# lenke182/flood-uav-video-segmentation

Hardware: AMD Instinct MI355X
Metric: segmentation FPS @713x713 (PSPNet-ResNet50 keyframe + linear interp, frame_delta=5) (higher is better)
Workload: dtype f32

## Files before the change

flood_uav_video_segmentation_amd/_lib.py:

```python
import ctypes
import os

import torch

_HERE = os.path.dirname(os.path.abspath(__file__))
LIB_PATH = os.path.join(_HERE, "libfloodseg.so")

c_float_p = ctypes.POINTER(ctypes.c_float)
c_void = ctypes.c_void_p
c_int = ctypes.c_int
c_i64 = ctypes.c_int64
c_f32 = ctypes.c_float


class FsConfig(ctypes.Structure):
    _fields_ = [("arch", c_int), ("layers", c_int), ("classes", c_int), ("patch", c_int), ("d_model", c_int),
                ("n_layers", c_int), ("dec_layers", c_int), ("image_size", c_int), ("flags", c_int), ("winograd_tile", c_int)]


ARCH_PSPNET = 0
ARCH_DEEPLABV3 = 1
ARCH_SEGMENTER = 2
OPT_NO_WINOGRAD = 1
OPT_NO_FUSED_HEAD = 2
# ... 87 lines not shown
    ("dual_conv", c_int, [c_void, c_int, c_void, c_int, c_void, c_void, c_void, c_void] + [c_int] * 12 + [c_void]),
    ("pyramid_pool", c_int, [c_void, c_int, c_void] + [c_int] * 4 + [c_void]),
    ("rowdot_batch", c_int, [c_int] + [c_void] * 6 + [c_int] * 5 + [c_void]),
    ("upsample_into", c_int, [c_void, c_int, c_int, c_void] + [c_int] * 6 + [c_void]),
    ("classifier_nchw", c_int, [c_void, c_int, c_void, c_void, c_void] + [c_int] * 4 + [c_void]),
    ("ppm_term_scratch_floats", ctypes.c_size_t, [c_int] * 3),
    ("ppm_term_classify", c_int, [c_void, c_int] + [c_void] * 7 + [c_int] * 5 + [c_void] * 3 + [c_int, c_void, c_void]),
    ("ppm_head_workspace_floats", ctypes.c_size_t, [c_int] * 3),
    ("ppm_head", c_int, [c_void, c_int, c_void, c_int] + [c_void] * 5 + [c_int] * 5 + [c_void] * 3 + [c_int, c_void, c_void]),
    ("block_match", c_int, [c_void, c_void] + [c_int] * 5 + [c_void, c_void, c_void]),
]

_EXT_HOOKS = [
    ("frame_prepare", c_int, [c_void, c_void, c_void] + [c_int] * 5 + [c_void, c_void, c_void, c_int, c_int, c_void]),
    ("frame_compose", c_int, [c_void, c_int, c_int, c_void, c_int, c_void, c_void, c_void] + [c_int] * 5 + [c_void, c_void, c_void] + [c_int] * 3 + [c_void]),
]
EXT_MAGIC = 0x4653455854414231

_EXT2_HOOKS = [
    ("block_match_modes", c_int, [c_void, c_void] + [c_int] * 7 + [c_void, c_void, c_void, c_void, c_void]),
    ("window_weights", c_int, [c_int, ctypes.POINTER(c_void), c_void, c_void, c_void]),
    ("seg_tail_weighted", c_int, [c_void, c_void, ctypes.POINTER(c_void), ctypes.POINTER(c_void)] + [c_int] * 9 + [c_void] * 4 + [c_int] * 4
     + [c_void, c_void, c_void]),
    ("crops_fuse_weighted", c_int, [c_void, c_void, c_void, c_int, ctypes.POINTER(c_int), ctypes.POINTER(c_int)] + [c_int] * 9
     + [c_void, c_void, c_int, c_int, c_void, c_void, c_void]),
    ("feat_tail_weighted", c_int, [c_void, c_void, c_int, c_int, c_int, ctypes.POINTER(c_void), ctypes.POINTER(c_void), c_int, c_int, c_void, c_int,
                                   c_int, c_int, c_int, c_void, c_void, c_void, c_void]),
    ("mask_confidence", c_int, [c_void] + [c_int] * 4 + [c_void, c_void, c_int, c_int, c_void]),
    ("canvas_confidence", c_int, [c_void] + [c_int] * 4 + [c_void, c_void, c_int, c_int, c_void]),
    ("frame_report", c_int, [c_void, c_void] + [c_int] * 5 + [c_void, c_void]),
    ("mask_regions", c_int, [c_void] + [c_int] * 5 + [c_void, c_void]),
    ("region_table", c_int, [c_void, c_void, c_void] + [c_int] * 6 + [c_void] * 5),
    ("region_filter", c_int, [c_void, c_void, c_void] + [c_int] * 6 + [c_void, c_void, c_void]),
]
EXT2_MAGIC = 0x4653455854414232


class FsTestApi(ctypes.Structure):
    _fields_ = [("size", ctypes.c_size_t)] + [(name, ctypes.CFUNCTYPE(res, *args)) for name, res, args in _HOOKS]


class FsExtApi(ctypes.Structure):
    _fields_ = [("magic", ctypes.c_uint64), ("size", ctypes.c_size_t)] + [(name, ctypes.CFUNCTYPE(res, *args)) for name, res, args in _EXT_HOOKS]


class FsHookTables(ctypes.Structure):
    _fields_ = [("test", FsTestApi), ("ext", FsExtApi)]


class FsExt2Api(ctypes.Structure):
    _fields_ = [("magic", ctypes.c_uint64), ("size", ctypes.c_size_t)] + [(name, ctypes.CFUNCTYPE(res, *args)) for name, res, args in _EXT2_HOOKS]


class FsHookTables2(ctypes.Structure):
    _fields_ = [("base", FsHookTables), ("ext2", FsExt2Api)]


class _Library:

    def __init__(self, cdll):
        self._cdll = cdll
        self._hooks = None
        self._ext = None
        self._ext2 = None

    def __getattr__(self, name):
# ... 108 lines not shown
```

flood_uav_video_segmentation_amd/csrc/conv_igemm.hip:

```cpp
#include "kernels.h"
#include "igemm_epilogue.h"

#include <algorithm>
#include <cstdlib>

namespace fs {

#define FS_DMA_PUBLISH() { __builtin_amdgcn_s_waitcnt(0x0070); __syncthreads(); }
constexpr int conv_split_rows(int BN, int waves) { return (BN / 16 + waves - 1) / waves * waves * 16; }
template <int BM, int BN, bool SPLIT, int WAVES = 4>
constexpr int conv_tile_lds_floats() { return 2 * (BM * 32 + (SPLIT ? 3 * conv_split_rows(BN, WAVES) * 16 : BN * 32)); }

template <int TM>
__device__ __forceinline__ void split_unit(int lvl, int pr, const f32x4 (&raw)[TM][2], float (&rq)[4 * TM][2], u32x4 (&ah)[TM][3], bool pin) {
    const int pi = pr / 4, pe = pr % 4;
    float x0 = lvl == 0 ? raw[pi][pe >> 1][2 * (pe & 1)] : rq[pr][0];
    float x1 = lvl == 0 ? raw[pi][pe >> 1][2 * (pe & 1) + 1] : rq[pr][1];
    unsigned pk = split_round(x0, x1);
    if (pin) asm volatile("" : "+v"(pk));
    ah[pi][lvl][pe] = pk;
    if (lvl < 2) {
        split_residue(pk, x0, x1);
        rq[pr][0] = x0;
        rq[pr][1] = x1;
// ... 294 lines not shown
#undef FS_DMA_ADVANCE
#undef FS_DMA_ALL
#undef FS_FRAGS
#undef FS_MMA

    if constexpr (SPLIT && !DUAL && BN == 96 && TM == 1) {
        const int Dm = p.kv_heads * 64;
        if (p.kv_k && n0 >= Dm) {
            const int kind = n0 >= 2 * Dm ? 2 : 1;
            igemm_epilogue_kv<TN>(acc, sc_n, sh_n, p, kind, em_base, en_base - kind * Dm, en_base < p.Cout, lane);
            return;
        }
    }
    if (!DUAL && p.res) {
        if (p.relu == 1) igemm_epilogue<1, true>(acc, rv, sc_n, sh_n, p, M, em_base, en_base);
        else if (p.relu == 2) igemm_epilogue<2, true>(acc, rv, sc_n, sh_n, p, M, em_base, en_base);
        else igemm_epilogue<0, true>(acc, rv, sc_n, sh_n, p, M, em_base, en_base);
    } else {
        if (p.relu == 1) igemm_epilogue<1, false>(acc, rv, sc_n, sh_n, p, M, em_base, en_base);
        else if (p.relu == 2) igemm_epilogue<2, false>(acc, rv, sc_n, sh_n, p, M, em_base, en_base);
        else igemm_epilogue<0, false>(acc, rv, sc_n, sh_n, p, M, em_base, en_base);
    }
#endif
}

template <int BM, int BN, int WGM = 2, int WGN = 2, bool DUAL = false, bool SPLIT = false>
__global__ __launch_bounds__(64 * WGM * WGN) void conv_igemm_dma_f32(ConvParams p, int tiles_m, int tiles_n) {
#if defined(__HIP_DEVICE_COMPILE__)
    constexpr int PM = 8;
    __shared__ __attribute__((aligned(1024))) float lds[conv_tile_lds_floats<BM, BN, SPLIT, WGM * WGN>()];
    const int nblk = gridDim.x, bid = blockIdx.x;
    const int q = nblk >> 3, rr = nblk & 7, xcd = bid & 7;
    const int lid = (xcd < rr ? xcd * (q + 1) : rr * (q + 1) + (xcd - rr) * q) + (bid >> 3);
    const int per_group = tiles_m * tiles_n;
    const int grp = lid / per_group;
    const int lig = lid - grp * per_group;
    const int panel = lig / (PM * tiles_n);
    const int within = lig - panel * (PM * tiles_n);
    const int prow = min(PM, tiles_m - panel * PM);
    const int m0 = (panel * PM + within % prow) * BM, n0 = (within / prow) * BN;
    p.in += (long long)grp * p.g_in;
    p.wgt += (long long)grp * p.g_wgt;
    if (SPLIT) p.wgt3 = (const char*)p.wgt3 + (long long)grp * p.g_wgt * 2;
    p.out += (long long)grp * p.g_out;
    p.kv_b = grp;
    conv_tile<BM, BN, WGM, WGN, DUAL, SPLIT>(p, m0, n0, lds);
#endif
}

namespace {
struct TileCfg { int bm, bn; const char* name; };
const TileCfg kTiles[7] = {{0, 0, "auto"}, {128, 128, "igemm128x128"}, {128, 64, "igemm128x64"},
                           {64, 64, "igemm64x64"}, {64, 128, "igemm64x128"}, {0, 0, nullptr}, {128, 96, "split128x96"}};
bool tile_id_ok(int tile) { return tile >= 0 && tile <= 6 && tile != 5; }

int pick_tile(const ConvParams& p) {
    const int M = p.B * p.Ho * p.Wo;
    const double eff[7] = {0, 1.00, 0.92, 0.80, 0.92, 0, 0.97};
    int best = 1;
    double best_t = 1e300;
    const int last = p.in2 ? 2 : p.wgt3 ? 3 : 4;
    for (int c = 1; c <= 6; ++c) {
        if (c > last && !(c == 6 && p.wgt3 && !p.in2 && p.Cout % 96 == 0)) continue;
        const int bm = kTiles[c].bm, bn = kTiles[c].bn;
        if (p.Cout < bn && bn > 64) continue;
        const long tiles = (long)cdiv(M, bm) * cdiv(p.Cout, bn) * (p.groups > 1 ? p.groups : 1);
        const long per_cu = (tiles + 255) / 256;
        const double t = (double)per_cu * bm * bn / (eff[c] * (per_cu >= 2 ? 1.0 : 0.8));
        if (t < best_t) { best_t = t; best = c; }
// ... 39 lines not shown
        FS_REQUIRE((p.H2 - 1) / p.stride2 + 1 == p.Ho && (p.W2 - 1) / p.stride2 + 1 == p.Wo, "conv_igemm: second operand %dx%d / stride %d does not give %dx%d",
                   p.H2, p.W2, p.stride2, p.Ho, p.Wo);
        FS_REQUIRE((int64_t)p.B * p.H2 * p.W2 * p.ld_in2 * 4 < (int64_t)1 << 31, "conv_igemm: second operand must be smaller than 2 GiB");
    }
    FS_REQUIRE(p.ld_in % 4 == 0 && p.ld_in >= p.Cin, "conv_igemm: bad ld_in=%d (Cin=%d)", p.ld_in, p.Cin);
    FS_REQUIRE(p.ld_out >= p.Cout, "conv_igemm: bad ld_out=%d (Cout=%d)", p.ld_out, p.Cout);
    FS_REQUIRE(((uintptr_t)p.in & 15) == 0 && ((uintptr_t)p.wgt & 15) == 0, "conv_igemm: unaligned operand");
    FS_REQUIRE(p.Ho == (p.H + 2 * p.pad - p.dil * (p.KH - 1) - 1) / p.stride + 1 &&
               p.Wo == (p.W + 2 * p.pad - p.dil * (p.KW - 1) - 1) / p.stride + 1,
               "conv_igemm: output geometry %dx%d inconsistent with input %dx%d", p.Ho, p.Wo, p.H, p.W);
    FS_REQUIRE(((int64_t)p.B * p.H * p.W * p.ld_in + ((int64_t)p.pad * p.W + p.pad) * p.ld_in) * 4 < (int64_t)1 << 31,
               "conv_igemm: input tensor must be smaller than 2 GiB");
    FS_REQUIRE((int64_t)p.Cout * std::max(p.ld_wgt, p.KH * p.KW * p.Cin + (p.in2 ? p.Cin2 : 0)) * 4 < (int64_t)1 << 31, "conv_igemm: filter bank must be smaller than 2 GiB");
    FS_REQUIRE(p.ld_wgt == 0 || (p.ld_wgt >= p.KH * p.KW * p.Cin + (p.in2 ? p.Cin2 : 0) && p.ld_wgt % 4 == 0), "conv_igemm: bad ld_wgt=%d", p.ld_wgt);
    FS_REQUIRE(p.KH * p.KW <= 32, "conv_igemm: at most 32 filter taps");
    FS_REQUIRE((int64_t)p.B * p.Ho * p.Wo * p.ld_out * 4 < (int64_t)1 << 31 && ((uintptr_t)p.out & 3) == 0,
               "conv_igemm: output tensor must be smaller than 2 GiB");
    FS_REQUIRE(p.res == nullptr || (int64_t)p.B * p.Ho * p.Wo * p.ld_res * 4 < (int64_t)1 << 31, "conv_igemm: residual tensor must be smaller than 2 GiB");
    if (!(p.res == nullptr || p.ld_res >= p.Cout)) return fail("conv_igemm: bad ld_res");
    return 0;
}
}

int launch_conv_igemm(const ConvParams& p, hipStream_t s, int tile) {
    FS_TRY(check_conv_params(p));
    FS_REQUIRE(tile_id_ok(tile), "conv_igemm: tile %d is not 0..4 or 6", tile);
    if (tile == 0) tile = pick_tile(p);
    FS_REQUIRE(tile < 6 || (p.wgt3 && !p.in2), "conv_igemm: tile 6 (128 x 96) exists on the split-operand route only");
    const int M = p.B * p.Ho * p.Wo;
    const int bm = kTiles[tile].bm, bn = kTiles[tile].bn;
    const int tm = cdiv(M, bm), tn = cdiv(p.Cout, bn);
    const int groups = p.groups > 1 ? p.groups : 1;
    FS_REQUIRE(groups == 1 || p.res == nullptr, "conv_igemm: grouped GEMM has no residual input");
    const dim3 grid(tm * tn * groups), block(256);
    if (p.kv_k) {
        const int Dm = p.kv_heads * 64;
        FS_REQUIRE(tile == 6 && p.wgt3 && !p.in2 && !p.res && p.KH == 1 && p.KW == 1 && p.stride == 1 && p.pad == 0 && p.relu == 0,
                   "conv_igemm: the K / V plane epilogue belongs to a plain Linear on the 128 x 96 split tile");
        FS_REQUIRE(p.kv_vt && p.kv_heads >= 1 && Dm % 96 == 0 && p.Cout == 3 * Dm && p.kv_N == M && p.kv_Npad % 32 == 0 && p.kv_Npad >= M &&
                       p.kv_Npad <= tm * bm && (int64_t)3 * p.kv_plane_bytes < (int64_t)1 << 31 &&
                       (int64_t)p.kv_plane_bytes == (int64_t)groups * p.kv_heads * p.kv_Npad * 128 && (((uintptr_t)p.kv_k | (uintptr_t)p.kv_vt) & 15) == 0,
                   "conv_igemm: bad K / V plane geometry (heads %d, tokens %d, padded %d)", p.kv_heads, p.kv_N, p.kv_Npad);
    }
    if (p.wgt3) {
        FS_REQUIRE(((uintptr_t)p.wgt3 & 15) == 0 && p.plane_bytes % 16 == 0 && (int64_t)3 * p.plane_bytes < (int64_t)1 << 31 && ldw_ok(p),
                   "conv_igemm: bad split filter bank (plane_bytes=%u)", p.plane_bytes);
        FS_REQUIRE((int64_t)groups * p.g_wgt * 2 <= (int64_t)p.plane_bytes, "conv_igemm: the groups' filters (%d x %lld) exceed a plane of the split bank", groups, p.g_wgt);
    }
    if (p.in2 && p.wgt3) {
        if (tile == 2) hipLaunchKernelGGL((conv_igemm_dma_f32<128, 64, 4, 1, true, true>), grid, block, 0, s, p, tm, tn);
        else if (tile == 1) hipLaunchKernelGGL((conv_igemm_dma_f32<128, 128, 4, 1, true, true>), grid, block, 0, s, p, tm, tn);
        else return fail("conv_igemm: concatenated-K launches use tile 1 or 2");
        FS_HIP(hipGetLastError());
        return 0;
    }
    if (p.in2) {
        if (tile == 2) hipLaunchKernelGGL((conv_igemm_dma_f32<128, 64, 2, 2, true>), grid, block, 0, s, p, tm, tn);
        else if (tile == 1) hipLaunchKernelGGL((conv_igemm_dma_f32<128, 128, 2, 2, true>), grid, block, 0, s, p, tm, tn);
        else return fail("conv_igemm: concatenated-K launches use tile 1 or 2");
        FS_HIP(hipGetLastError());
        return 0;
    }
    if (p.wgt3) {
        switch (tile) {
            case 1: hipLaunchKernelGGL((conv_igemm_dma_f32<128, 128, 4, 1, false, true>), grid, block, 0, s, p, tm, tn); break;
            case 2: hipLaunchKernelGGL((conv_igemm_dma_f32<128, 64, 4, 1, false, true>), grid, block, 0, s, p, tm, tn); break;
            case 3: hipLaunchKernelGGL((conv_igemm_dma_f32<64, 64, 2, 2, false, true>), grid, block, 0, s, p, tm, tn); break;
// ... 22 lines not shown
```

flood_uav_video_segmentation_amd/csrc/kernels.h:

```cpp
#pragma once
#include "common.h"

namespace fs {

struct ConvParams {
    const float* in;    int ld_in;
    const float* wgt;
    int ld_wgt;
    const float* scale;
    const float* shift;
    const float* res;   int ld_res;
    float* out;         int ld_out;
    int B, H, W, Cin;
    int Ho, Wo, Cout;
    int KH, KW, stride, pad, dil;
    const float* in2;   int ld_in2;
    int Cin2, stride2, H2, W2;
    int relu;
    int res_touch;
    int korder;
    int groups;
    long long g_in, g_wgt, g_out;
    const void* wgt3;
    unsigned plane_bytes;
    unsigned short* kv_k;
    unsigned short* kv_vt;
    int kv_N, kv_Npad, kv_heads;
    unsigned kv_plane_bytes;
    int kv_b;
};
int launch_conv_igemm(const ConvParams& p, hipStream_t s, int tile = 0);
const char* conv_igemm_tile_name(const ConvParams& p, int tile = 0);
int launch_split_bf16x3(const float* w, long long n, void* planes, hipStream_t s);

static inline int conv_out_size(int in, int k, int stride, int pad, int dil) { return (in + 2 * pad - dil * (k - 1) - 1) / stride + 1; }
static inline ConvParams conv2d_params(const float* in, int ld_in, const float* wgt, const float* scale, const float* shift, const float* res, int ld_res,
                                       float* out, int ld_out, int B, int H, int W, int Cin, int Cout, int KH, int KW, int stride, int pad, int dil,
                                       int relu, int korder) {
    ConvParams p{};
    p.in = in; p.ld_in = ld_in; p.wgt = wgt; p.scale = scale; p.shift = shift; p.res = res; p.ld_res = ld_res; p.out = out; p.ld_out = ld_out;
    p.B = B; p.H = H; p.W = W; p.Cin = Cin; p.Cout = Cout;
    p.Ho = conv_out_size(H, KH, stride, pad, dil);
    p.Wo = conv_out_size(W, KW, stride, pad, dil);
    p.KH = KH; p.KW = KW; p.stride = stride; p.pad = pad; p.dil = dil; p.relu = relu; p.korder = korder;
    return p;
}
static inline ConvParams gemm_params(const float* in, int ld_in, const float* w, float* out, int ld_out, int rows, int K, int N) {
    return conv2d_params(in, ld_in, w, nullptr, nullptr, nullptr, 0, out, ld_out, 1, rows, 1, K, N, 1, 1, 1, 0, 1, 0, 0);
}
static inline void attach_planes(ConvParams& p, const void* planes, size_t elems) {
    p.wgt3 = planes;
    p.plane_bytes = (unsigned)(elems * 2);
}

struct FrameSrc {
// ... 252 lines not shown
```

flood_uav_video_segmentation_amd/csrc/net.h:

```cpp
#pragma once
#include <map>
#include <memory>
#include <string>
#include <vector>

#include "../../include/floodseg.h"
#include "kernels.h"

namespace fs {

struct RawTensor {
    float* d = nullptr;
    std::vector<int64_t> shape;
    int64_t numel() const {
        int64_t n = 1;
        for (auto s : shape) n *= s;
        return n;
    }
};

struct WinoBank {
    float* U4 = nullptr;
    float* U6 = nullptr;
    float* U3 = nullptr;
// ... 97 lines not shown
    bool res_touch = true;
    std::map<const float*, std::pair<void*, size_t>> split_banks;
    int device = 0;

    float* buf[4] = {nullptr, nullptr, nullptr, nullptr};
    size_t buf_elems = 0;
    float* small = nullptr;
    size_t small_elems = 0;

    bool profiling = false;
    std::vector<fs::ProfRec> prof;

    int feat_channels() const {
        if (cfg.arch == FS_ARCH_SEGMENTER) return cfg.d_model;
        return cfg.arch == FS_ARCH_PSPNET ? 4096 : 2048;
    }
};

namespace fs {
int net_create(const fs_config* cfg, fs_handle* out);
int net_destroy(fs_handle h);
int check_device(fs_net* h, const char* what);
int net_load_weight(fs_handle h, const char* name, const float* data, const int64_t* shape, int ndim, int on_device,
                    hipStream_t s);
int net_finalize(fs_handle h, hipStream_t s);
int net_feature_shape(fs_handle h, int H, int W, int* C, int* fh, int* fw);
size_t net_workspace_bytes(fs_handle h, int B, int H, int W);
int net_reserve(fs_handle h, int B, int H, int W, hipStream_t s);
size_t net_reserved_bytes(fs_handle h);
int net_encoder(fs_handle h, const FrameSrc& src, int B, int H, int W, float* out_nhwc, hipStream_t s);
int net_segment(fs_handle h, const FrameSrc& src, int B, int H, int W, float* out_nchw, hipStream_t s);
int net_decoder(fs_handle h, const float* feat, int B, int fh, int fw, float* out_nchw, hipStream_t s);
int net_profile_dump(fs_handle h, char* buf, size_t n);

int dev_alloc(fs_net* h, float** p, size_t elems);
int ws_grow(fs_net* h, float** p, size_t* have, size_t need, bool zero);
int split_attach(fs_net* h, const float* bank, size_t elems, hipStream_t s);
void split_use(const fs_net* h, ConvParams& p);

int linear_splits(int K, int N, int rows_per_image, int act, bool split_route);
ConvParams linear_params(const float* in, const float* w, const float* bias, const float* res, float* out, int rows, int K, int N, int act,
                         bool res_touch);
ConvParams linear_splitk_params(const float* in, const float* w, float* part, int rows, int K, int N, int split);
ConvParams linear_qkv_params(const float* in, const float* w, const float* bias, float* out, int B, int tokens, int D, float* planes);
ConvParams dual_conv_params(const float* a, int ld_a, const float* b, int ld_b, const float* wgt, const float* shift, float* out, int ld_out, int B,
                            int Ho, int Wo, int Cin, int Cin2, int H2, int W2, int stride2, int Cout, int relu);
ConvParams ppm_z_params(const float* reduced, const float* zw, float* zbuf, int B, int Cr, int Cout9);
int pyramid_pool(fs_net* h, const float* feat, int ld_feat, float* pooled, int B, int H, int W, int C, const int bins[4], hipStream_t s);
int conv_winograd(fs_net* h, const std::string& name, const float* in, int ld_in, const float* U, const void* U3, unsigned plane_bytes, float* V,
                  float* M, const float* scale, const float* shift, float* out, int ld_out, int B, int H, int W, int Cin, int Cout, int dil,
                  int relu, int mt, hipStream_t s);
int vit_reserve(fs_handle h, int B, int H, int W, hipStream_t s);
int fetch(fs_net* h, const std::string& name, const RawTensor** out);
int prof_begin(fs_net* h, const std::string& name, const char* kernel, double flops, double bytes, hipStream_t s);
int prof_end(fs_net* h, hipStream_t s);
int run_igemm(fs_net* h, const std::string& name, const ConvParams& p, double flops, double bytes, hipStream_t s, int tile = 0);
int vit_finalize(fs_handle h, hipStream_t s);
int vit_feature_shape(fs_handle h, int H, int W, int* C, int* fh, int* fw);
int vit_encoder(fs_handle h, const FrameSrc& src, int B, int H, int W, float* out_tokens, hipStream_t s);
int vit_decoder(fs_handle h, const float* tokens, int B, int gh, int gw, float* out_nchw, hipStream_t s);
}
```

flood_uav_video_segmentation_amd/csrc/net.hip:

```cpp
#include "net.h"

#include <cmath>
#include <cstdarg>
#include <cstring>

namespace fs {

std::string& last_error() {
    static thread_local std::string e;
    return e;
}
int fail(const char* fmt, ...) {
    char buf[1024];
    va_list ap;
    va_start(ap, fmt);
    vsnprintf(buf, sizeof(buf), fmt, ap);
    va_end(ap);
    last_error() = buf;
    return 1;
}

int dev_alloc(fs_net* h, float** p, size_t elems) {
    FS_HIP(hipMalloc(reinterpret_cast<void**>(p), std::max<size_t>(elems, 4) * sizeof(float)));
    h->owned.push_back(*p);
// ... 552 lines not shown
    size_t wino = 0;
    if (h->deep_stem) {
        FS_TRY(reserve_conv(h, h->stem[1], B, g.H1, g.W1, s, &wino));
        FS_TRY(reserve_conv(h, h->stem[2], B, g.H1, g.W1, s, &wino));
    }
    int curH = g.H2, curW = g.W2;
    for (const Bottleneck& blk : h->blocks) {
        FS_TRY(reserve_conv(h, blk.c2, B, curH, curW, s, &wino));
        curH = blk.c2.out_size(curH);
        curW = blk.c2.out_size(curW);
    }
    if (psp) {
        FS_TRY(reserve_conv(h, h->use_fused_head ? h->cls_main : h->cls_conv, B, fh, fw, s, &wino));
        FS_TRY(reserve_conv(h, h->cls_conv, B, fh, fw, s, &wino));
    } else {
        for (int i = 1; i < 4; ++i) FS_TRY(reserve_conv(h, h->aspp[i], B, fh, fw, s, &wino));
        FS_TRY(reserve_conv(h, h->head_conv, B, fh, fw, s, &wino));
    }
    return ws_grow(h, &h->wino_ws, &h->wino_ws_elems, wino, false);
}

size_t net_reserved_bytes(fs_handle h) {
    if (!h) return 0;
    return (4 * h->buf_elems + h->small_elems + h->seg_feat_elems + h->wino_ws_elems + h->vit_ws_elems + h->pos_elems + h->bank_elems) * sizeof(float);
}

ConvParams dual_conv_params(const float* a, int ld_a, const float* b, int ld_b, const float* wgt, const float* shift, float* out, int ld_out, int B,
                            int Ho, int Wo, int Cin, int Cin2, int H2, int W2, int stride2, int Cout, int relu) {
    ConvParams p = conv2d_params(a, ld_a, wgt, nullptr, shift, nullptr, 0, out, ld_out, B, Ho, Wo, Cin, Cout, 1, 1, 1, 0, 1, relu, 0);
    p.in2 = b; p.ld_in2 = ld_b; p.Cin2 = Cin2; p.stride2 = stride2; p.H2 = H2; p.W2 = W2;
    return p;
}

ConvParams ppm_z_params(const float* reduced, const float* zw, float* zbuf, int B, int Cr, int Cout9) {
    const int rows = B * 36;
    ConvParams p = gemm_params(reduced, Cr, zw, zbuf, Cout9, rows, Cr, Cout9);
    p.groups = 4;
    p.g_in = (long long)rows * Cr;
    p.g_wgt = (long long)Cout9 * Cr;
    p.g_out = (long long)rows * Cout9;
    return p;
}

int pyramid_pool(fs_net* h, const float* feat, int ld_feat, float* pooled, int B, int H, int W, int C, const int bins[4], hipStream_t s) {
    size_t pool_off[4];
    {
        size_t po = 0;
        for (int i = 0; i < 4; ++i) {
            pool_off[i] = po;
            po += (size_t)B * bins[i] * bins[i] * C;
        }
    }
    const double bytes = 4.0 * B * H * W * C;
    if (H % 6 == 0 && W % 6 == 0 && bins[0] == 1 && bins[1] == 2 && bins[2] == 3 && bins[3] == 6) {
        FS_TRY(prof_begin(h, "ppm.pool6+combine", "adaptive_avgpool", 0, bytes, s));
        FS_TRY(launch_adaptive_avgpool(feat, ld_feat, pooled + pool_off[3], B, H, W, C, 6, s));
        FS_TRY(launch_ppm_pool_combine(pooled + pool_off[3], pooled + pool_off[0], pooled + pool_off[1], pooled + pool_off[2], B, C, s));
        FS_TRY(prof_end(h, s));
        return 0;
    }
    for (int i = 0; i < 4; ++i) {
        FS_TRY(prof_begin(h, "ppm.pool" + std::to_string(bins[i]), "adaptive_avgpool", 0, bytes, s));
        FS_TRY(launch_adaptive_avgpool(feat, ld_feat, pooled + pool_off[i], B, H, W, C, bins[i], s));
        FS_TRY(prof_end(h, s));
    }
    return 0;
}

namespace {
int pyramid_reduce(fs_net* h, const float* feat, int ld_feat, int B, int H, int W, hipStream_t s) {
    float* pooled = h->small;
    float* reduced = h->small + (size_t)B * 50 * 2048;
    FS_TRY(pyramid_pool(h, feat, ld_feat, pooled, B, H, W, 2048, h->bins, s));
// ... 130 lines not shown
    FS_REQUIRE(out_nchw && B >= 1 && H >= 1 && W >= 1, "fs_segment_forward: bad arguments (B=%d H=%d W=%d)", B, H, W);
    FS_TRY(check_frames(src, B, "fs_segment_forward"));
    int C = 0, fh = 0, fw = 0;
    if (h->cfg.arch != FS_ARCH_PSPNET || !h->use_fused_head) {
        FS_TRY(net_feature_shape(h, H, W, &C, &fh, &fw));
        const size_t need = h->cfg.arch == FS_ARCH_SEGMENTER ? (size_t)B * (fh * fw + 1) * C : (size_t)B * fh * fw * C;
        FS_TRY(ws_grow(h, &h->seg_feat, &h->seg_feat_elems, need, false));
        FS_TRY(net_encoder(h, src, B, H, W, h->seg_feat, s));
        return net_decoder(h, h->seg_feat, B, fh, fw, out_nchw, s);
    }
    FS_REQUIRE(H >= 33 && W >= 33, "fs_segment_forward: bad arguments (B=%d H=%d W=%d)", B, H, W);
    const Geometry g = geometry(h, H, W);
    fh = g.H3;
    fw = g.W3;
    FS_TRY(ensure_workspace(h, std::max(encoder_buf_elems(h, B, H, W), ppm_term_scratch_floats(B, fh, h->cls_main.Cout)), small_elems_for(B)));
    float* feat = nullptr;
    FS_TRY(encoder_core(h, src, B, H, W, nullptr, &feat, s));
    hipStream_t ps = s;
    FS_TRY(pyramid_reduce(h, feat, 2048, B, fh, fw, ps));
    float *T = nullptr, *R = nullptr;
    for (int i = 0; i < 4; ++i)
        if (h->buf[i] != feat) {
            R = T;
            T = h->buf[i];
        }
    FS_REQUIRE(ppm_term_scratch_floats(B, fh, h->cls_main.Cout) <= h->buf_elems, "fs_segment_forward: workspace too small for the pyramid term");
    const int K = h->cfg.classes, O = h->cls_main.Cout;
    const size_t px = (size_t)B * fh * fw;
    float* reduced = h->small + (size_t)B * 50 * 2048;
    float* zbuf = reduced + (size_t)4 * B * 36 * 512;
    const float* Z[4];
    {
        const ConvBN& z = h->ppm_z[0];
        ConvParams p = ppm_z_params(reduced, z.w, zbuf, B, 512, z.Cout);
        split_use(h, p);
        FS_TRY(run_igemm(h, "decoder.0.weight[:, ppm]", p, 2.0 * B * 50 * 512.0 * z.Cout, 4.0 * (4.0 * z.Cout * 512 + B * 50.0 * (512 + z.Cout)), ps));
        for (int i = 0; i < 4; ++i) Z[i] = zbuf + (size_t)i * p.g_out;
    }
    ConvBN raw = h->cls_main;
    raw.scale = raw.shift = nullptr;
    raw.relu = 0;
    FS_TRY(run_conv(h, raw, feat, 2048, B, fh, fw, T, O, nullptr, 0, s));
    FS_TRY(prof_begin(h, "decoder.0.pyramid_term+decoder.4", "ppm_term_classify", 2.0 * px * O * (24.0 + K), 4.0 * px * O, s));
    FS_TRY(launch_ppm_term_classify(T, O, Z, h->bins, R, h->cls_main.scale, h->cls_main.shift, B, fh, fw, O, 1, h->cls_w, h->cls_b, out_nchw, K, s));
    return prof_end(h, s);
}

int net_decoder(fs_handle h, const float* feat, int B, int fh, int fw, float* out_nchw, hipStream_t s) {
    FS_REQUIRE(h && h->finalized, "fs_decoder_forward: network not finalized");
    FS_TRY(check_device(h, "fs_decoder_forward"));
    if (h->cfg.arch == FS_ARCH_SEGMENTER) return vit_decoder(h, feat, B, fh, fw, out_nchw, s);
    FS_REQUIRE(feat && out_nchw && B >= 1 && fh >= 1 && fw >= 1, "fs_decoder_forward: bad arguments");
    const int K = h->cfg.classes;
    const size_t px = (size_t)B * fh * fw;
    if (h->cfg.arch == FS_ARCH_PSPNET) {
        FS_TRY(ensure_workspace(h, px * 512, small_elems_for(B)));
        float* T = h->buf[0];
        FS_TRY(run_conv(h, h->cls_conv, feat, 4096, B, fh, fw, T, 512, nullptr, 0, s));
        FS_TRY(prof_begin(h, "decoder.4", "classifier_nchw", 2.0 * px * 512.0 * K, 4.0 * px * 512.0, s));
        FS_TRY(launch_classifier_nchw(T, 512, h->cls_w, h->cls_b, out_nchw, B, fh * fw, 512, K, s));
        return prof_end(h, s);
    }
    FS_TRY(ensure_workspace(h, px * 1280, small_elems_for(B)));
    float *cat = h->buf[0], *P = h->buf[1], *Q = h->buf[2];
    for (int i = 0; i < 4; ++i) FS_TRY(run_conv(h, h->aspp[i], feat, 2048, B, fh, fw, cat + 256 * i, 1280, nullptr, 0, s));
    float* pooled = h->small;
    float* reduced = h->small + (size_t)B * 2048;
    FS_TRY(prof_begin(h, "aspp.pool", "adaptive_avgpool", 0, 4.0 * px * 2048.0, s));
    if (fh % 6 == 0 && fw % 6 == 0) {
        float* cells = h->small + (size_t)B * 4096;
        float* spare = cells + (size_t)B * 36 * 2048;
        FS_TRY(launch_adaptive_avgpool(feat, 2048, cells, B, fh, fw, 2048, 6, s));
        FS_TRY(launch_ppm_pool_combine(cells, pooled, spare, spare + (size_t)B * 4 * 2048, B, 2048, s));
    } else {
        FS_TRY(launch_adaptive_avgpool(feat, 2048, pooled, B, fh, fw, 2048, 1, s));
    }
    FS_TRY(prof_end(h, s));
    FS_TRY(prof_begin(h, h->aspp_pool.name, "rowdot_1x1", 2.0 * B * 2048.0 * 256.0, 4.0 * 2048.0 * 256.0, s));
// ... 32 lines not shown
```

flood_uav_video_segmentation_amd/csrc/net_ops.hip:

```cpp
#include "interp.h"
#include "kernels.h"
#include "split.h"

#include <type_traits>

namespace fs {

template <int CPT >
__global__ __launch_bounds__(256) void stem_conv_kernel(StemParams p) {
    extern __shared__ __attribute__((aligned(16))) float wlds[];
    const int taps = p.KH * p.KW * 3;
    for (int i = threadIdx.x; i < taps * p.Cout; i += 256) wlds[i] = p.wgt[i];
    __syncthreads();

    const int groups = p.Cout / CPT;
    const int ppb = 256 / groups;
    const int cg = threadIdx.x % groups;
    const int M = p.B * p.Ho * p.Wo;
    const int m = blockIdx.x * ppb + threadIdx.x / groups;
    if (m >= M) return;
    const int hw = p.Ho * p.Wo;
    const int b = m / hw;
    const int rem = m - b * hw;
    const int oy = rem / p.Wo, ox = rem - oy * p.Wo;
// ... 376 lines not shown
__global__ __launch_bounds__(256) void ppm_pool_combine_kernel(const float* __restrict__ cell_mean , float* __restrict__ out1,
                                                               float* __restrict__ out2, float* __restrict__ out3, int B, int C) {
    const int64_t total = (int64_t)B * C;
    for (int64_t i = (int64_t)blockIdx.x * 256 + threadIdx.x; i < total; i += (int64_t)gridDim.x * 256) {
        const int c = (int)(i % C), b = (int)(i / C);
        const float* m = cell_mean + (size_t)b * 36 * C + c;
        float s3[9], s2[4] = {0.f, 0.f, 0.f, 0.f}, s1 = 0.f;
#pragma unroll
        for (int k = 0; k < 9; ++k) s3[k] = 0.f;
#pragma unroll
        for (int y = 0; y < 6; ++y)
#pragma unroll
            for (int x = 0; x < 6; ++x) {
                const float v = m[(size_t)(y * 6 + x) * C];
                s3[(y / 2) * 3 + x / 2] += v;
                s2[(y / 3) * 2 + x / 3] += v;
                s1 += v;
            }
#pragma unroll
        for (int k = 0; k < 9; ++k) out3[((size_t)b * 9 + k) * C + c] = s3[k] * 0.25f;
#pragma unroll
        for (int k = 0; k < 4; ++k) out2[((size_t)b * 4 + k) * C + c] = s2[k] * (1.f / 9.f);
        out1[(size_t)b * C + c] = s1 * (1.f / 36.f);
    }
}

int launch_ppm_pool_combine(const float* cell_mean, float* out1, float* out2, float* out3, int B, int C, hipStream_t s) {
    const int64_t total = (int64_t)B * C;
    hipLaunchKernelGGL(ppm_pool_combine_kernel, dim3((unsigned)cdiv64(total, 256)), dim3(256), 0, s, cell_mean, out1, out2, out3, B, C);
    FS_HIP(hipGetLastError());
    return 0;
}

template <int KV >
__global__ __launch_bounds__(256) void rowdot_1x1_kernel(RowdotBatch pb, int ld_in, int ld_out, int K, int N, int relu) {
    const RowdotProblem& q = pb.p[blockIdx.z];
    const int lane = threadIdx.x & 63;
    const int n = blockIdx.x * 4 + (threadIdx.x >> 6);
    if (n >= N) return;
    const int M = q.M;
    const int per = (M + gridDim.y - 1) / gridDim.y;
    const int m_begin = blockIdx.y * per, m_end = min(M, (int)(blockIdx.y + 1) * per);
    if (m_begin >= m_end) return;
    f32x4 w[KV];
#pragma unroll
    for (int i = 0; i < KV; ++i) w[i] = *reinterpret_cast<const f32x4*>(q.wgt + (size_t)n * K + (i * 64 + lane) * 4);
    const float sc = q.scale ? q.scale[n] : 1.f, sh = q.shift ? q.shift[n] : 0.f;
    for (int m = m_begin; m < m_end; ++m) {
        float acc = 0.f;
#pragma unroll
        for (int i = 0; i < KV; ++i) {
            const f32x4 x = *reinterpret_cast<const f32x4*>(q.in + (size_t)m * ld_in + (i * 64 + lane) * 4);
            acc += x[0] * w[i][0] + x[1] * w[i][1] + x[2] * w[i][2] + x[3] * w[i][3];
        }
#pragma unroll
        for (int off = 32; off > 0; off >>= 1) acc += __shfl_xor(acc, off, 64);
        if (lane == 0) {
            float y = acc * sc + sh;
            if (relu) y = fmaxf(y, 0.f);
            q.out[(size_t)m * ld_out + n] = y;
        }
    }
}

int launch_rowdot_1x1_batch(const RowdotBatch& pb, int nprob, int ld_in, int ld_out, int K, int N, int relu, hipStream_t s) {
    FS_REQUIRE(K % 256 == 0 && K <= 4096, "rowdot_1x1: K=%d must be a multiple of 256 and <= 4096", K);
    FS_REQUIRE(nprob >= 1 && nprob <= 4, "rowdot_1x1: 1..4 problems per launch");
    int mmax = 1;
    for (int i = 0; i < nprob; ++i) mmax = std::max(mmax, pb.p[i].M);
    const dim3 grid(cdiv(N, 4), std::max(1, std::min(12, mmax / 6)), nprob), block(256);
#define FS_ROWDOT(KV)                                                                                             \
    case KV:                                                                                                      \
        hipLaunchKernelGGL((rowdot_1x1_kernel<KV>), grid, block, 0, s, pb, ld_in, ld_out, K, N, relu);            \
        break;
    switch (K / 256) {
        FS_ROWDOT(1) FS_ROWDOT(2) FS_ROWDOT(3) FS_ROWDOT(4) FS_ROWDOT(5) FS_ROWDOT(6) FS_ROWDOT(7) FS_ROWDOT(8)
        FS_ROWDOT(9) FS_ROWDOT(10) FS_ROWDOT(11) FS_ROWDOT(12) FS_ROWDOT(13) FS_ROWDOT(14) FS_ROWDOT(15) FS_ROWDOT(16)
        default: return fail("rowdot_1x1: unsupported K");
    }
#undef FS_ROWDOT
    FS_HIP(hipGetLastError());
    return 0;
}

int launch_rowdot_1x1(const float* in, int ld_in, const float* wgt, const float* scale, const float* shift, float* out,
                      int ld_out, int M, int K, int N, int relu, hipStream_t s) {
    RowdotBatch pb{};
    pb.p[0] = RowdotProblem{in, wgt, scale, shift, out, M};
    return launch_rowdot_1x1_batch(pb, 1, ld_in, ld_out, K, N, relu, s);
}

int launch_upsample_into(const float* in, int hi, int wi, float* out, int ld_out, int B, int Ho, int Wo, int C,
                         int align_corners, hipStream_t s) {
    FS_REQUIRE(C % 4 == 0 && ld_out % 4 == 0 && ((uintptr_t)out & 15) == 0, "upsample_into: C/ld_out must be multiples of 4");
    return launch_resize_bilinear_nhwc(in, C, B, C, hi, wi, out, ld_out, Ho, Wo, align_corners, s, 256 * 32);
}

__global__ __launch_bounds__(256) void classifier_nchw_kernel(const float* __restrict__ in, int ld_in, const float* __restrict__ wgt,
                                                              const float* __restrict__ bias, float* __restrict__ out, int B,
                                                              int HW, int C, int K) {
    extern __shared__ __attribute__((aligned(16))) float wl[];
    for (int i = threadIdx.x; i < K * C; i += 256) wl[i] = wgt[i];
    __syncthreads();
    const int l16 = threadIdx.x & 15;
    const int64_t M = (int64_t)B * HW;
    const int64_t m = (int64_t)blockIdx.x * 16 + (threadIdx.x >> 4);
    const int64_t mc = m < M ? m : M - 1;
    const float* x = in + (size_t)mc * ld_in;
    for (int k0 = 0; k0 < K; k0 += 8) {
        float acc[8];
// ... 332 lines not shown
```

Before: 1244.

## Size PPM grouped GEMM per-bin rows and restructure rowdot 1x1 kernel

The pyramid-pooling grouped GEMM now carries per-group row counts (B*bin^2), so each bin launches only the row tiles it needs instead of padding every group to 36 rows. The rowdot 1x1 kernel now computes several output channels and two rows per wave, reusing each input load across channels. It splits rows into fixed chunks across problems and stages results in LDS for vectorised stores. A poison hook is also added for testing that skipped rows are never read. The cost is more register pressure in rowdot and extra index arithmetic in the igemm tile mapping.

```diff
diff --git a/flood_uav_video_segmentation_amd/_lib.py b/flood_uav_video_segmentation_amd/_lib.py
--- a/flood_uav_video_segmentation_amd/_lib.py
+++ b/flood_uav_video_segmentation_amd/_lib.py
@@ -143,6 +143,7 @@
     ("mask_regions", c_int, [c_void] + [c_int] * 5 + [c_void, c_void]),
     ("region_table", c_int, [c_void, c_void, c_void] + [c_int] * 6 + [c_void] * 5),
     ("region_filter", c_int, [c_void, c_void, c_void] + [c_int] * 6 + [c_void, c_void, c_void]),
+    ("pyramid_poison", c_int, [c_void, c_int, c_void]),
 ]
 EXT2_MAGIC = 0x4653455854414232
 
diff --git a/flood_uav_video_segmentation_amd/csrc/conv_igemm.hip b/flood_uav_video_segmentation_amd/csrc/conv_igemm.hip
--- a/flood_uav_video_segmentation_amd/csrc/conv_igemm.hip
+++ b/flood_uav_video_segmentation_amd/csrc/conv_igemm.hip
@@ -350,9 +350,17 @@
     const int nblk = gridDim.x, bid = blockIdx.x;
     const int q = nblk >> 3, rr = nblk & 7, xcd = bid & 7;
     const int lid = (xcd < rr ? xcd * (q + 1) : rr * (q + 1) + (xcd - rr) * q) + (bid >> 3);
-    const int per_group = tiles_m * tiles_n;
-    const int grp = lid / per_group;
-    const int lig = lid - grp * per_group;
+    int grp, lig;
+    if (p.g_rows[0] > 0) {
+        const int t0 = ((p.g_rows[0] + BM - 1) / BM) * tiles_n, t1 = ((p.g_rows[1] + BM - 1) / BM) * tiles_n, t2 = ((p.g_rows[2] + BM - 1) / BM) * tiles_n;
+        grp = lid < t0 ? 0 : lid < t0 + t1 ? 1 : lid < t0 + t1 + t2 ? 2 : 3;
+        lig = lid - (grp > 0 ? t0 : 0) - (grp > 1 ? t1 : 0) - (grp > 2 ? t2 : 0);
+        tiles_m = (((grp == 0 ? p.g_rows[0] : grp == 1 ? p.g_rows[1] : grp == 2 ? p.g_rows[2] : p.g_rows[3]) + BM - 1) / BM);
+    } else {
+        const int per_group = tiles_m * tiles_n;
+        grp = lid / per_group;
+        lig = lid - grp * per_group;
+    }
     const int panel = lig / (PM * tiles_n);
     const int within = lig - panel * (PM * tiles_n);
     const int prow = min(PM, tiles_m - panel * PM);
@@ -458,7 +466,16 @@
     const int tm = cdiv(M, bm), tn = cdiv(p.Cout, bn);
     const int groups = p.groups > 1 ? p.groups : 1;
     FS_REQUIRE(groups == 1 || p.res == nullptr, "conv_igemm: grouped GEMM has no residual input");
-    const dim3 grid(tm * tn * groups), block(256);
+    int row_tiles = tm * groups;
+    if (p.g_rows[0] > 0) {
+        FS_REQUIRE(groups >= 2 && groups <= 4 && !p.kv_k, "conv_igemm: per-group row counts belong to a plain grouped GEMM of 2..4 groups");
+        row_tiles = 0;
+        for (int g = 0; g < 4; ++g) {
+            FS_REQUIRE(g < groups ? p.g_rows[g] >= 1 && p.g_rows[g] <= M : p.g_rows[g] == 0, "conv_igemm: group %d has %d rows of %d", g, p.g_rows[g], M);
+            row_tiles += cdiv(p.g_rows[g], bm);
+        }
+    }
+    const dim3 grid(row_tiles * tn), block(256);
     if (p.kv_k) {
         const int Dm = p.kv_heads * 64;
         FS_REQUIRE(tile == 6 && p.wgt3 && !p.in2 && !p.res && p.KH == 1 && p.KW == 1 && p.stride == 1 && p.pad == 0 && p.relu == 0,
diff --git a/flood_uav_video_segmentation_amd/csrc/kernels.h b/flood_uav_video_segmentation_amd/csrc/kernels.h
--- a/flood_uav_video_segmentation_amd/csrc/kernels.h
+++ b/flood_uav_video_segmentation_amd/csrc/kernels.h
@@ -21,6 +21,7 @@
     int korder;
     int groups;
     long long g_in, g_wgt, g_out;
+    int g_rows[4];
     const void* wgt3;
     unsigned plane_bytes;
     unsigned short* kv_k;
diff --git a/flood_uav_video_segmentation_amd/csrc/net.h b/flood_uav_video_segmentation_amd/csrc/net.h
--- a/flood_uav_video_segmentation_amd/csrc/net.h
+++ b/flood_uav_video_segmentation_amd/csrc/net.h
@@ -153,6 +153,7 @@
 int net_segment(fs_handle h, const FrameSrc& src, int B, int H, int W, float* out_nchw, hipStream_t s);
 int net_decoder(fs_handle h, const float* feat, int B, int fh, int fw, float* out_nchw, hipStream_t s);
 int net_profile_dump(fs_handle h, char* buf, size_t n);
+int net_pyramid_poison(fs_handle h, int B, hipStream_t s);
 
 int dev_alloc(fs_net* h, float** p, size_t elems);
 int ws_grow(fs_net* h, float** p, size_t* have, size_t need, bool zero);
@@ -166,7 +167,7 @@
 ConvParams linear_qkv_params(const float* in, const float* w, const float* bias, float* out, int B, int tokens, int D, float* planes);
 ConvParams dual_conv_params(const float* a, int ld_a, const float* b, int ld_b, const float* wgt, const float* shift, float* out, int ld_out, int B,
                             int Ho, int Wo, int Cin, int Cin2, int H2, int W2, int stride2, int Cout, int relu);
-ConvParams ppm_z_params(const float* reduced, const float* zw, float* zbuf, int B, int Cr, int Cout9);
+ConvParams ppm_z_params(const float* reduced, const float* zw, float* zbuf, int B, int Cr, int Cout9, const int bins[4]);
 int pyramid_pool(fs_net* h, const float* feat, int ld_feat, float* pooled, int B, int H, int W, int C, const int bins[4], hipStream_t s);
 int conv_winograd(fs_net* h, const std::string& name, const float* in, int ld_in, const float* U, const void* U3, unsigned plane_bytes, float* V,
                   float* M, const float* scale, const float* shift, float* out, int ld_out, int B, int H, int W, int Cin, int Cout, int dil,
diff --git a/flood_uav_video_segmentation_amd/csrc/net.hip b/flood_uav_video_segmentation_amd/csrc/net.hip
--- a/flood_uav_video_segmentation_amd/csrc/net.hip
+++ b/flood_uav_video_segmentation_amd/csrc/net.hip
@@ -608,13 +608,14 @@
     return p;
 }
 
-ConvParams ppm_z_params(const float* reduced, const float* zw, float* zbuf, int B, int Cr, int Cout9) {
+ConvParams ppm_z_params(const float* reduced, const float* zw, float* zbuf, int B, int Cr, int Cout9, const int bins[4]) {
     const int rows = B * 36;
     ConvParams p = gemm_params(reduced, Cr, zw, zbuf, Cout9, rows, Cr, Cout9);
     p.groups = 4;
     p.g_in = (long long)rows * Cr;
     p.g_wgt = (long long)Cout9 * Cr;
     p.g_out = (long long)rows * Cout9;
+    for (int i = 0; i < 4; ++i) p.g_rows[i] = B * bins[i] * bins[i];
     return p;
 }
 
@@ -811,7 +812,7 @@
     const float* Z[4];
     {
         const ConvBN& z = h->ppm_z[0];
-        ConvParams p = ppm_z_params(reduced, z.w, zbuf, B, 512, z.Cout);
+        ConvParams p = ppm_z_params(reduced, z.w, zbuf, B, 512, z.Cout, h->bins);
         split_use(h, p);
         FS_TRY(run_igemm(h, "decoder.0.weight[:, ppm]", p, 2.0 * B * 50 * 512.0 * z.Cout, 4.0 * (4.0 * z.Cout * 512 + B * 50.0 * (512 + z.Cout)), ps));
         for (int i = 0; i < 4; ++i) Z[i] = zbuf + (size_t)i * p.g_out;
@@ -823,6 +824,16 @@
     FS_TRY(prof_begin(h, "decoder.0.pyramid_term+decoder.4", "ppm_term_classify", 2.0 * px * O * (24.0 + K), 4.0 * px * O, s));
     FS_TRY(launch_ppm_term_classify(T, O, Z, h->bins, R, h->cls_main.scale, h->cls_main.shift, B, fh, fw, O, 1, h->cls_w, h->cls_b, out_nchw, K, s));
     return prof_end(h, s);
+}
+
+int net_pyramid_poison(fs_handle h, int B, hipStream_t s) {
+    FS_REQUIRE(h && h->finalized && B >= 1, "pyramid_poison: bad arguments");
+    FS_TRY(check_device(h, "pyramid_poison"));
+    FS_REQUIRE(h->buf_elems > 0 && h->small && small_elems_for(B) <= h->small_elems, "pyramid_poison: no workspace for %d frames yet", B);
+    for (int i = 0; i < 4; ++i) FS_HIP(hipMemsetAsync(h->buf[i], 0xFF, h->buf_elems * sizeof(float), s));
+    float* zbuf = h->small + (size_t)B * 50 * 2048 + (size_t)4 * B * 36 * 512;
+    FS_HIP(hipMemsetAsync(zbuf, 0xFF, (size_t)4 * B * 36 * 9 * 512 * sizeof(float), s));
+    return 0;
 }
 
 int net_decoder(fs_handle h, const float* feat, int B, int fh, int fw, float* out_nchw, hipStream_t s) {
diff --git a/flood_uav_video_segmentation_amd/csrc/net_ops.hip b/flood_uav_video_segmentation_amd/csrc/net_ops.hip
--- a/flood_uav_video_segmentation_amd/csrc/net_ops.hip
+++ b/flood_uav_video_segmentation_amd/csrc/net_ops.hip
@@ -432,33 +432,76 @@
     return 0;
 }
 
-template <int KV >
-__global__ __launch_bounds__(256) void rowdot_1x1_kernel(RowdotBatch pb, int ld_in, int ld_out, int K, int N, int relu) {
-    const RowdotProblem& q = pb.p[blockIdx.z];
-    const int lane = threadIdx.x & 63;
-    const int n = blockIdx.x * 4 + (threadIdx.x >> 6);
-    if (n >= N) return;
-    const int M = q.M;
-    const int per = (M + gridDim.y - 1) / gridDim.y;
-    const int m_begin = blockIdx.y * per, m_end = min(M, (int)(blockIdx.y + 1) * per);
-    if (m_begin >= m_end) return;
-    f32x4 w[KV];
-#pragma unroll
-    for (int i = 0; i < KV; ++i) w[i] = *reinterpret_cast<const f32x4*>(q.wgt + (size_t)n * K + (i * 64 + lane) * 4);
-    const float sc = q.scale ? q.scale[n] : 1.f, sh = q.shift ? q.shift[n] : 0.f;
-    for (int m = m_begin; m < m_end; ++m) {
-        float acc = 0.f;
-#pragma unroll
-        for (int i = 0; i < KV; ++i) {
-            const f32x4 x = *reinterpret_cast<const f32x4*>(q.in + (size_t)m * ld_in + (i * 64 + lane) * 4);
-            acc += x[0] * w[i][0] + x[1] * w[i][1] + x[2] * w[i][2] + x[3] * w[i][3];
-        }
-#pragma unroll
-        for (int off = 32; off > 0; off >>= 1) acc += __shfl_xor(acc, off, 64);
+constexpr int ROWDOT_PER = 8;
+constexpr int ROWDOT_NC = 4;
+constexpr int ROWDOT_RG = 2;
+constexpr int ROWDOT_MAXR = 16;
+static_assert(ROWDOT_PER >= 1 && ROWDOT_PER <= ROWDOT_MAXR, "a chunk's rows must fit the staging block");
+struct RowdotGrid { int first[5]; int per[4]; };
+
+template <int KV , int NC, int RG>
+__global__ __launch_bounds__(256) void rowdot_1x1_kernel(RowdotBatch pb, RowdotGrid g, int ld_in, int ld_out, int K, int N, int relu) {
+    __shared__ __attribute__((aligned(16))) float red[ROWDOT_MAXR][4 * NC];
+    const int ch = blockIdx.y;
+    const int pi = ch < g.first[1] ? 0 : ch < g.first[2] ? 1 : ch < g.first[3] ? 2 : 3;
+    const RowdotProblem& q = pb.p[pi];
+    const int lane = threadIdx.x & 63, wv = threadIdx.x >> 6;
+    const int m_begin = (ch - g.first[pi]) * g.per[pi], m_end = min(q.M, m_begin + g.per[pi]);
+    const int n0 = blockIdx.x * 4 * NC;
+    f32x4 w[NC][KV];
+    float sc[NC], sh[NC];
+#pragma unroll
+    for (int c = 0; c < NC; ++c) {
+        const int n = min(n0 + wv * NC + c, N - 1);
+#pragma unroll
+        for (int i = 0; i < KV; ++i) w[c][i] = *reinterpret_cast<const f32x4*>(q.wgt + (size_t)n * K + (i * 64 + lane) * 4);
+        sc[c] = q.scale ? q.scale[n] : 1.f;
+        sh[c] = q.shift ? q.shift[n] : 0.f;
+    }
+    for (int m0 = m_begin; m0 < m_end; m0 += RG) {
+        float acc[RG][NC];
+#pragma unroll
+        for (int r = 0; r < RG; ++r) {
+            const int m = min(m0 + r, m_end - 1);
+#pragma unroll
+            for (int c = 0; c < NC; ++c) acc[r][c] = 0.f;
+#pragma unroll
+            for (int i = 0; i < KV; ++i) {
+                const f32x4 x = *reinterpret_cast<const f32x4*>(q.in + (size_t)m * ld_in + (i * 64 + lane) * 4);
+#pragma unroll
+                for (int c = 0; c < NC; ++c) acc[r][c] += x[0] * w[c][i][0] + x[1] * w[c][i][1] + x[2] * w[c][i][2] + x[3] * w[c][i][3];
+            }
+        }
+#pragma unroll
+        for (int off = 32; off > 0; off >>= 1)
+#pragma unroll
+            for (int r = 0; r < RG; ++r)
+#pragma unroll
+                for (int c = 0; c < NC; ++c) acc[r][c] += __shfl_xor(acc[r][c], off, 64);
         if (lane == 0) {
-            float y = acc * sc + sh;
-            if (relu) y = fmaxf(y, 0.f);
-            q.out[(size_t)m * ld_out + n] = y;
+#pragma unroll
+            for (int r = 0; r < RG; ++r)
+                if (m0 + r < m_end) {
+#pragma unroll
+                    for (int c = 0; c < NC; ++c) {
+                        float y = acc[r][c] * sc[c] + sh[c];
+                        if (relu) y = fmaxf(y, 0.f);
+                        red[m0 + r - m_begin][wv * NC + c] = y;
+                    }
+                }
+        }
+    }
+    __syncthreads();
+    const int rows = m_end - m_begin;
+    if ((int)threadIdx.x < rows * NC) {
+        const int r = threadIdx.x / NC, qd = threadIdx.x - r * NC;
+        const int n = n0 + qd * 4;
+        float* o = q.out + (size_t)(m_begin + r) * ld_out + n;
+        if (n + 4 <= N && (ld_out & 3) == 0 && ((uintptr_t)q.out & 15) == 0) {
+            *reinterpret_cast<f32x4*>(o) = *reinterpret_cast<const f32x4*>(&red[r][qd * 4]);
+        } else {
+            for (int e = 0; e < 4; ++e)
+                if (n + e < N) o[e] = red[r][qd * 4 + e];
         }
     }
 }
@@ -466,16 +509,27 @@
 int launch_rowdot_1x1_batch(const RowdotBatch& pb, int nprob, int ld_in, int ld_out, int K, int N, int relu, hipStream_t s) {
     FS_REQUIRE(K % 256 == 0 && K <= 4096, "rowdot_1x1: K=%d must be a multiple of 256 and <= 4096", K);
     FS_REQUIRE(nprob >= 1 && nprob <= 4, "rowdot_1x1: 1..4 problems per launch");
-    int mmax = 1;
-    for (int i = 0; i < nprob; ++i) mmax = std::max(mmax, pb.p[i].M);
-    const dim3 grid(cdiv(N, 4), std::max(1, std::min(12, mmax / 6)), nprob), block(256);
-#define FS_ROWDOT(KV)                                                                                             \
-    case KV:                                                                                                      \
-        hipLaunchKernelGGL((rowdot_1x1_kernel<KV>), grid, block, 0, s, pb, ld_in, ld_out, K, N, relu);            \
+    RowdotGrid g{};
+    RowdotBatch q = pb;
+    for (int i = 0; i < 4; ++i) {
+        if (i >= nprob) q.p[i] = RowdotProblem{};
+        const int M = q.p[i].M > 0 ? q.p[i].M : 0;
+        const int chunks = cdiv(M, ROWDOT_PER);
+        g.per[i] = chunks ? cdiv(M, chunks) : 0;
+        g.first[i + 1] = g.first[i] + chunks;
+    }
+    if (g.first[4] == 0) return 0;
+    FS_REQUIRE(g.first[4] <= 65535, "rowdot_1x1: too many rows for one launch");
+    const int NCW = K / 256 <= 8 ? ROWDOT_NC : 1;
+    const dim3 grid(cdiv(N, 4 * NCW), g.first[4]), block(256);
+#define FS_ROWDOT(KV, NC)                                                                                                 \
+    case KV:                                                                                                              \
+        hipLaunchKernelGGL((rowdot_1x1_kernel<KV, NC, ROWDOT_RG>), grid, block, 0, s, q, g, ld_in, ld_out, K, N, relu);   \
         break;
     switch (K / 256) {
-        FS_ROWDOT(1) FS_ROWDOT(2) FS_ROWDOT(3) FS_ROWDOT(4) FS_ROWDOT(5) FS_ROWDOT(6) FS_ROWDOT(7) FS_ROWDOT(8)
-        FS_ROWDOT(9) FS_ROWDOT(10) FS_ROWDOT(11) FS_ROWDOT(12) FS_ROWDOT(13) FS_ROWDOT(14) FS_ROWDOT(15) FS_ROWDOT(16)
+        FS_ROWDOT(1, ROWDOT_NC) FS_ROWDOT(2, ROWDOT_NC) FS_ROWDOT(3, ROWDOT_NC) FS_ROWDOT(4, ROWDOT_NC)
+        FS_ROWDOT(5, ROWDOT_NC) FS_ROWDOT(6, ROWDOT_NC) FS_ROWDOT(7, ROWDOT_NC) FS_ROWDOT(8, ROWDOT_NC)
+        FS_ROWDOT(9, 1) FS_ROWDOT(10, 1) FS_ROWDOT(11, 1) FS_ROWDOT(12, 1) FS_ROWDOT(13, 1) FS_ROWDOT(14, 1) FS_ROWDOT(15, 1) FS_ROWDOT(16, 1)
         default: return fail("rowdot_1x1: unsupported K");
     }
 #undef FS_ROWDOT
```

Result: no change. 1237 (-0.6%).
